# raider99k/UNINA-YOLO-DLA

Measured on NVIDIA B200. Metric: images/sec @640x640 (forward + DFL decode + NMS), higher is better.
Workload: dtype bf16

## Files before the change

unina-yolo-dla_b200/csrc/api.cu:

```cuda
#include <cstdarg>
#include <cstdlib>
#include <memory>
#include <mutex>
#include <set>
#include <utility>

#include "camera.cuh"
#include "common.cuh"

namespace uyd {

static thread_local char g_err[512] = "";

void set_error(const char *fmt, ...) {
  va_list ap;
  va_start(ap, fmt);
  vsnprintf(g_err, sizeof(g_err), fmt, ap);
  va_end(ap);
}

int smem_optin_impl(const void *kernel, int bytes) {
  static std::mutex mu;
  static std::set<std::pair<const void *, int>> done;
  int dev = 0;
// ... 47 lines not shown

struct ClsArgs {
  const __nv_bfloat16 *in;
  float *out;
  const __nv_bfloat16 *wdw;
  const uint32_t *wfrag;
  const float *bias;
  int n, h, w, in_pitch, out_pitch, nc, tiles_x, tiles_y;
};
bool cls_branch_supported(int cin, int mid, int nc, int h, int w, int in_pitch, int in_coff, int out_pitch, int out_coff);
void cls_branch_pack(int cin, int nc, const float *const w[5], const float *const b[5], std::vector<__nv_bfloat16> &wdw,
                     std::vector<uint32_t> &frags, std::vector<float> &bias);
int cls_branch_launch(int cin, const ClsArgs &a, cudaStream_t s);

struct ChainConv;
ChainConv *chain_new();
void chain_delete(ChainConv *);
bool chain_supported(int cin, int n1, int n2, int in_pitch, int in_coff);
size_t chain_w1_bytes(int cin, int n1, bool depthwise);
size_t chain_w2_bytes(int n1, int n2);
void chain_pack_w1(int cin, int n1, bool depthwise, const float *w, void *dst_host);
void chain_pack_w2(int n1, int n2, const float *w, void *dst_host);
int chain_prepare(ChainConv *cc, int cin, int n1, int n2, void *in_base, int in_pitch, int h, int w, int max_batch,
                  void *w1_dev, void *w2_dev, const float *bias1, const float *bias2, int relu2, int final_kind, int nc,
                  const float *w3_dev, const float *bias3_dev, void *out_base, int out_pitch, int out_f32, int a_total,
                  int a_off, int y_ch0, int no, float stride_px, int dw1);
int chain_launch(const ChainConv *cc, int nb, float *y, int sm_count, cudaStream_t s);

struct StemArgs {
  const void *in;
  __nv_bfloat16 *out;
  const uint32_t *wfrag;
  const float *bias;
  int n, ih, iw, oh, ow, out_pitch, u8, pw;
  CamFrames f;
};
bool stem_fused_supported(int c0, int c1, int ih, int iw, int out_pitch, int out_coff);
void stem_fused_pack(const float *w0, const float *b0, const float *w1, const float *b1, const float *w2, const float *b2,
                     std::vector<uint32_t> &frags, std::vector<float> &bias);
int stem_fused_launch(const StemArgs &a, cudaStream_t s);

// ... 21 lines not shown
  std::vector<float> b_host;
  void *w_dev = nullptr;
  float *b_dev = nullptr;
  TcConv *tc = nullptr;
  std::vector<float> m_host;
  float *m_dev = nullptr;
  float out_scale = 0.f;
  int out_kind = 0;
  std::vector<unsigned char> w2_host;
  void *w2_dev = nullptr;
  int nc = 0;
  uyd_chain chain{};
  ChainConv *cc = nullptr;
  std::vector<float> b2_host, w3_host, b3_host;
  float *b2_dev = nullptr, *w3_dev = nullptr, *b3_dev = nullptr;
  bool quant = false;
  int buf = -1, coff = 0, c = 0, out_buf = -1, out_coff = 0;
};

struct uyd_plan {
  uyd_ctx *ctx = nullptr;
  int max_batch = 0;
  bool finalized = false;
  std::vector<Buffer> bufs;
  std::vector<Op> ops;
  std::vector<int> heads, head_strides;
  int reg_max = 16, nc = 0;
  float dfl_amax = 0.f;
  int in_c = 0, in_h = 0, in_w = 0;
  size_t bytes = 0;
// ... 50 lines not shown
}

extern "C" int uyd_plan_destroy(uyd_plan *plan) {
  if (!plan) return UYD_OK;
  uyd::DeviceGuard guard(plan->ctx->device);
  for (Op &o : plan->ops) {
    if (o.w_dev) cudaFree(o.w_dev);
    if (o.b_dev) cudaFree(o.b_dev);
    if (o.m_dev) cudaFree(o.m_dev);
    if (o.w2_dev) cudaFree(o.w2_dev);
    if (o.tc) tc_delete(o.tc);
    if (o.cc) chain_delete(o.cc);
    if (o.b2_dev) cudaFree(o.b2_dev);
    if (o.w3_dev) cudaFree(o.w3_dev);
    if (o.b3_dev) cudaFree(o.b3_dev);
  }
  if (plan->arena) cudaFree(plan->arena);
  for (cudaEvent_t e : plan->timed_ev) cudaEventDestroy(e);
  delete plan;
  return UYD_OK;
}

extern "C" int uyd_plan_add_buffer(uyd_plan *plan, int h, int w, int c, int dtype, int *id) {
  UYD_REQUIRE(plan && id && h > 0 && w > 0 && c > 0, UYD_E_ARG, "uyd_plan_add_buffer: bad arguments");
  UYD_REQUIRE(!plan->finalized, UYD_E_STATE, "plan already finalized");
  UYD_REQUIRE(dtype == UYD_BF16 || dtype == UYD_F32 || dtype == UYD_S8, UYD_E_ARG, "unknown dtype %d", dtype);
  Buffer b;
  b.h = h; b.w = w; b.c = c; b.dtype = dtype;
  plan->bufs.push_back(b);
  *id = (int)plan->bufs.size() - 1;
// ... 372 lines not shown
    UYD_REQUIRE(b.dtype == UYD_F32 && b.c == 4 * reg_max + nc, UYD_E_ARG, "head buffer %d must be fp32 with %d channels", i,
                4 * reg_max + nc);
  }
  plan->heads.assign(head_bufs, head_bufs + nl);
  plan->head_strides.assign(strides, strides + nl);
  plan->reg_max = reg_max;
  plan->nc = nc;
  return UYD_OK;
}

static void *slice_ptr(const uyd_plan *p, int buf, int coff) {
  const Buffer &b = p->bufs[buf];
  return (char *)b.ptr + (size_t)coff * b.elem_bytes();
}

extern "C" int uyd_plan_finalize(uyd_plan *plan) {
  UYD_REQUIRE(plan && !plan->finalized, UYD_E_STATE, "plan missing or already finalized");
  UYD_REQUIRE(!plan->arena, UYD_E_STATE, "uyd_plan_finalize failed before on this plan: destroy it (uyd_plan_destroy frees the partial allocations)");
  uyd::DeviceGuard guard(plan->ctx->device);
  UYD_CUDA(guard.err);
  size_t total = 0;
  std::vector<size_t> offs;
  for (Buffer &b : plan->bufs) {
    offs.push_back(total);
    total += (b.bytes_per_image() * plan->max_batch + 1023) & ~(size_t)1023;
  }
  UYD_CUDA(cudaMalloc(&plan->arena, total ? total : 1024));
  UYD_CUDA(cudaMemset(plan->arena, 0, total ? total : 1024));
  for (size_t i = 0; i < plan->bufs.size(); ++i) plan->bufs[i].ptr = (char *)plan->arena + offs[i];
  plan->bytes = total;
  const int halo_fallback = env_int("UYD_TC_NO_HALO", 0);
  const int bo_mode = env_int("UYD_TC_BASE_OFFSET", 0);
  const int stages = env_int("UYD_TC_STAGES", 0);
  const int halo_pitch = env_int("UYD_TC_HALO_PITCH", 10);
  for (Op &o : plan->ops) {
    if (o.kind != OP_CONV && o.kind != OP_CONV_S8 && o.kind != OP_C3K && o.kind != OP_CLS && o.kind != OP_CHAIN && o.kind != OP_STEM2) continue;
    UYD_CUDA(cudaMalloc(&o.w_dev, o.w_host.size()));
    UYD_CUDA(cudaMemcpy(o.w_dev, o.w_host.data(), o.w_host.size(), cudaMemcpyHostToDevice));
    UYD_CUDA(cudaMalloc((void **)&o.b_dev, o.b_host.size() * 4));
    UYD_CUDA(cudaMemcpy(o.b_dev, o.b_host.data(), o.b_host.size() * 4, cudaMemcpyHostToDevice));
    plan->bytes += o.w_host.size() + o.b_host.size() * 4;
    o.w_host.clear();
    o.w_host.shrink_to_fit();
    if (o.kind == OP_CLS) {
      UYD_CUDA(cudaMalloc(&o.w2_dev, o.w2_host.size()));
      UYD_CUDA(cudaMemcpy(o.w2_dev, o.w2_host.data(), o.w2_host.size(), cudaMemcpyHostToDevice));
      continue;
    }
    if (o.kind == OP_CHAIN) {
      const uyd_chain &d = o.chain;
      UYD_CUDA(cudaMalloc(&o.w2_dev, o.w2_host.size()));
      UYD_CUDA(cudaMemcpy(o.w2_dev, o.w2_host.data(), o.w2_host.size(), cudaMemcpyHostToDevice));
      UYD_CUDA(cudaMalloc((void **)&o.b2_dev, o.b2_host.size() * 4));
      UYD_CUDA(cudaMemcpy(o.b2_dev, o.b2_host.data(), o.b2_host.size() * 4, cudaMemcpyHostToDevice));
      if (!o.w3_host.empty()) {
        UYD_CUDA(cudaMalloc((void **)&o.w3_dev, o.w3_host.size() * 4));
        UYD_CUDA(cudaMemcpy(o.w3_dev, o.w3_host.data(), o.w3_host.size() * 4, cudaMemcpyHostToDevice));
        UYD_CUDA(cudaMalloc((void **)&o.b3_dev, o.b3_host.size() * 4));
        UYD_CUDA(cudaMemcpy(o.b3_dev, o.b3_host.data(), o.b3_host.size() * 4, cudaMemcpyHostToDevice));
      }
      const Buffer &ib = plan->bufs[d.in_buf];
      void *out = nullptr;
      int out_pitch = 0, out_f32 = 0;
      if (d.out_buf >= 0) {
        out = slice_ptr(plan, d.out_buf, d.out_coff);
        out_pitch = plan->bufs[d.out_buf].c;
        out_f32 = plan->bufs[d.out_buf].dtype == UYD_F32;
      }
      o.cc = chain_new();
      int e = chain_prepare(o.cc, d.cin, d.n1, d.n2, slice_ptr(plan, d.in_buf, d.in_coff), ib.c, ib.h, ib.w, plan->max_batch, o.w_dev,
                            o.w2_dev, o.b_dev, o.b2_dev, d.relu2, d.final_kind, d.nc, o.w3_dev, o.b3_dev, out, out_pitch, out_f32,
                            d.a_total, d.a_off, d.y_ch0, d.no, d.stride_px, d.dw1);
      if (e) return e;
      continue;
    }
    if (o.kind == OP_C3K || o.kind == OP_STEM2) continue;
    if (o.kind == OP_CONV_S8) {
      UYD_CUDA(cudaMalloc((void **)&o.m_dev, o.m_host.size() * 4));
      UYD_CUDA(cudaMemcpy(o.m_dev, o.m_host.data(), o.m_host.size() * 4, cudaMemcpyHostToDevice));
      if (o.use_tc) {
        const uyd_conv &d = o.conv;
        const Buffer &ib = plan->bufs[d.in_buf], &ob = plan->bufs[d.out_buf];
        o.tc = tc_new();
        const void *res = d.res_buf >= 0 ? slice_ptr(plan, d.res_buf, d.res_coff) : nullptr;
        int e = tc_prepare(o.tc, d, slice_ptr(plan, d.in_buf, d.in_coff), ib.c, ib.h, ib.w, plan->max_batch,
                           slice_ptr(plan, d.out_buf, d.out_coff), ob.c, 0, res, d.res_buf >= 0 ? plan->bufs[d.res_buf].c : 0, o.w_dev,
                           o.b_dev, halo_fallback ? 2 : -1, bo_mode, stages, 1, o.m_dev, o.out_scale, o.out_kind, halo_pitch);
// ... 269 lines not shown
    by = (double)b.h * b.w * o.c * 3;
    snprintf(text, text_len, "quantize c%d %dx%d bf16->s8", o.c, b.h, b.w);
  } else if (o.kind == OP_STEM2) {
    const Buffer &b = plan->bufs[o.out_buf];
    fl = 2.0 * (4.0 * b.h * b.w * 16 * 27 + (double)b.h * b.w * 32 * 144 + (o.c ? (double)b.h * b.w * 16 * 32 : 0.0));
    by = 16.0 * b.h * b.w * 3 * 4 + (double)b.h * b.w * (o.c ? 16 : 32) * 2;
    snprintf(text, text_len, "stem2 3->16 k3 s2 + 16->32 k3 s2%s fused -> %dx%d", o.c ? " + 32->16 k1" : "", b.h, b.w);
  } else if (o.kind == OP_CHAIN) {
    const uyd_chain &d = o.chain;
    const Buffer &b = plan->bufs[d.in_buf];
    const double px = (double)b.h * b.w;
    fl = 2.0 * px * ((d.dw1 ? 9.0 * d.cin : 9.0 * d.cin * d.n1) + (double)d.n1 * d.n2 + (d.final_kind == UYD_CHAIN_PW3 ? (double)d.n2 * d.nc : 0.0));
    const double dec = d.final_kind == UYD_CHAIN_DFL ? 16 : (d.final_kind == UYD_CHAIN_PW3 ? 4.0 * d.nc : 0);
    const double rawb = d.out_buf >= 0 ? (d.final_kind == UYD_CHAIN_PW3 ? 4.0 * d.nc : d.n2 * (double)plan->bufs[d.out_buf].elem_bytes()) : 0;
    by = px * (d.cin * 2.0 + rawb + (d.out_buf >= 0 && d.final_kind != UYD_CHAIN_STORE ? 0 : dec));
    snprintf(text, text_len, "chain %s%d->%d k3 + %d->%d k1 + %s %dx%d tc", d.dw1 ? "dw" : "", d.cin, d.n1, d.n1, d.n2,
             d.final_kind == UYD_CHAIN_DFL ? "dfl" : (d.final_kind == UYD_CHAIN_PW3 ? "pw3" : "store"), b.h, b.w);
  } else if (o.kind == OP_CLS) {
    const Buffer &b = plan->bufs[o.buf];
    const double c = o.c;
    fl = 2.0 * b.h * b.w * (9 * c + c * 32 + 9 * 32 + 32 * 32 + 32 * o.nc);
    by = (double)b.h * b.w * (c * 2 + o.nc * 4);
    snprintf(text, text_len, "cls_branch_fused c%d %dx%d (5 convs)", o.c, b.h, b.w);
  } else if (o.kind == OP_C3K) {
    const Buffer &b = plan->bufs[o.buf];
    const double c = o.c, h = c / 2;
    fl = 2.0 * b.h * b.w * (2 * c * h + 4 * 9 * h * h + c * c);
    by = (double)b.h * b.w * c * 2 * 2;
    snprintf(text, text_len, "%s c%d %dx%d (7 convs)", o.quant ? "c3k_fused_s8" : "c3k_fused", o.c, b.h, b.w);
  } else if (o.kind == OP_SPPF) {
    const Buffer &b = plan->bufs[o.buf];
    by = (double)b.h * b.w * o.c * 2 * 4;
// ... 52 lines not shown
```

unina-yolo-dla_b200/csrc/conv_chain.cu:

```cuda
#include <cstdlib>

#include "common.cuh"
#include "tc_ptx.cuh"

namespace uyd {

enum { CH_STORE = 0, CH_PW3 = 2, CH_DFL = 3 };

struct ChainParams {
  int H, W, n0, nb;
  int tiles_x, tiles_y;
  long long total_tiles;
  int ncb, cb_bytes;
  int N1, N2;
  int c2;
  int stages;
  uint32_t blk_bytes, tx_bytes, w1_bytes, w2_bytes, a2_bytes;
  uint32_t idesc1, idesc2, layout1, layout2;
  int relu2, final_kind, nc;
  const float *bias1, *bias2, *bias3, *w3;
  const float *dw_w;
  void *out;
  int out_pitch, out_f32;
  float *y;
  int a_total, a_off, y_ch0, no;
  float stride_px;
  unsigned tpi, m_tpi, m_tx;
  long long *dbg;
};

namespace {

constexpr int kNG = 3;
constexpr int kChainThreads = 128 + 128 * kNG;
constexpr int kHaloRows = 18, kTileH = 16, kTileW = 8, kHaloPitch = kTileW + 2;

__device__ __forceinline__ float sigmoidf_(float x) { return __fdividef(1.0f, 1.0f + __expf(-x)); }

__device__ __forceinline__ float2 ffma2(float2 a, float2 b, float2 c) {
  float2 d;
  asm("{\n\t.reg .b64 ra, rb, rc, rd;\n\tmov.b64 ra, {%2, %3};\n\tmov.b64 rb, {%4, %5};\n\tmov.b64 rc, {%6, %7};\n\t"
      "fma.rn.f32x2 rd, ra, rb, rc;\n\tmov.b64 {%0, %1}, rd;\n\t}"
      : "=f"(d.x), "=f"(d.y)
      : "f"(a.x), "f"(a.y), "f"(b.x), "f"(b.y), "f"(c.x), "f"(c.y));
  return d;
}

__device__ __forceinline__ void load_bias16(const float *s, float (&v)[16]) {
#pragma unroll
  for (int i = 0; i < 4; ++i) {
    const float4 q = reinterpret_cast<const float4 *>(s)[i];
    v[4 * i] = q.x; v[4 * i + 1] = q.y; v[4 * i + 2] = q.z; v[4 * i + 3] = q.w;
  }
}

__device__ __forceinline__ void stamp(const ChainParams &p, int it, int slot, int lane) {
  if (p.dbg && blockIdx.x == 0 && lane == 0 && it < 64) p.dbg[(slot >> 3) * 512 + it * 8 + (slot & 7)] = clock64();
}

template <int KS1, int KS2, bool DW>
__global__ void __launch_bounds__(kChainThreads, 1) conv_chain_kernel(const __grid_constant__ CUtensorMap tm_in,
                                                                      const __grid_constant__ CUtensorMap tm_w1,
                                                                      const __grid_constant__ CUtensorMap tm_w2,
                                                                      const ChainParams p) {
  extern __shared__ unsigned char smem_dyn[];
  const uint32_t raw = smem_u32(smem_dyn);
  const uint32_t base = (raw + 1023u) & ~1023u;
  const uint32_t w1_s = base;
  const uint32_t w2_s = w1_s + ((p.w1_bytes + 1023u) & ~1023u);
  const uint32_t a2_s = w2_s + ((p.w2_bytes + 1023u) & ~1023u);
  const uint32_t a_s = a2_s + (uint32_t)kNG * p.a2_bytes;
  const uint32_t bar0 = a_s + (uint32_t)p.stages * p.blk_bytes;
  const uint32_t full0 = bar0, empty0 = bar0 + 64, wfull = bar0 + 128;
  const uint32_t tfull1 = bar0 + 136, tempty1 = bar0 + 168, a2full = bar0 + 200, tfull2 = bar0 + 232, tempty2 = bar0 + 264;
  const uint32_t slot = bar0 + 296;
  uint32_t *slot_ptr = reinterpret_cast<uint32_t *>(smem_dyn + (slot - raw));
  float *fs = reinterpret_cast<float *>(smem_dyn + (bar0 + 320u - raw));
  float *bias1_s = fs, *bias2_s = fs + 128, *bias3_s = fs + 256, *w3_s = fs + 264;

  const int warp = threadIdx.x >> 5, lane = threadIdx.x & 31;
  uint32_t tmem_cols = 32;
  while (tmem_cols < (uint32_t)kNG * (uint32_t)(p.N1 + p.N2)) tmem_cols <<= 1;

  if (threadIdx.x == 0) {
    for (int s = 0; s < p.stages; ++s) {
      mbar_init(full0 + 8u * s, 1);
      mbar_init(empty0 + 8u * s, DW ? 128 : 1);
    }
    mbar_init(wfull, 1);
    for (int g = 0; g < kNG; ++g) {
      mbar_init(tfull1 + 8u * g, 1);
      mbar_init(tempty1 + 8u * g, 128);
      mbar_init(a2full + 8u * g, 128);
      mbar_init(tfull2 + 8u * g, 1);
      mbar_init(tempty2 + 8u * g, 128);
    }
    fence_barrier_init();
    mbar_expect_tx(wfull, p.w1_bytes + p.w2_bytes);
    const int nblk = DW ? 0 : p.ncb * 9;
    for (int i = 0; i < nblk; ++i) tma_load_2d(w1_s + (uint32_t)i * p.N1 * p.cb_bytes, &tm_w1, wfull, 0, i * p.N1);
    tma_load_2d(w2_s, &tm_w2, wfull, 0, 0);
  }
  griddep_trigger();
  for (int i = threadIdx.x; i < 128; i += kChainThreads) {
    bias1_s[i] = i < p.N1 ? p.bias1[i] : 0.f;
    bias2_s[i] = i < p.N2 ? p.bias2[i] : 0.f;
  }
  if (p.final_kind == CH_PW3) {
    for (int i = threadIdx.x; i < 8 * 64; i += kChainThreads) {
      const int k = i >> 3, c = i & 7;
      w3_s[((k >> 1) * 8 + c) * 2 + (k & 1)] = (c < p.nc && k < p.N2) ? p.w3[c * p.N2 + k] : 0.f;
    }
    if (threadIdx.x < 8) bias3_s[threadIdx.x] = threadIdx.x < p.nc ? p.bias3[threadIdx.x] : 0.f;
  }
  if (warp == 1) tmem_alloc(slot, tmem_cols);
  tc_fence_before();
  __syncthreads();
  tc_fence_after();
  const uint32_t tmem_base = *slot_ptr;
  griddep_wait();

  const int stages = p.stages;
  const uint32_t blk_bytes = p.blk_bytes, cb_bytes = p.cb_bytes;
  const uint32_t cb2_bytes = (uint32_t)p.N1 * 2u;

  if (warp == 0) {
    int stage = 0;
    uint32_t phase = 0;
// ... 3 lines not shown
      const unsigned ty = fastdiv(t, (unsigned)p.tiles_x, p.m_tx);
      const int n = p.n0 + (int)img;
      const int y0 = (int)ty * kTileH, x0 = (int)(t - ty * (unsigned)p.tiles_x) * kTileW;
      for (int j = 0; j < p.ncb; ++j) {
        mbar_wait(empty0 + 8u * stage, phase ^ 1u);
        if (lane == 0) {
          const uint32_t fb = full0 + 8u * stage;
          mbar_expect_tx(fb, p.tx_bytes);
          tma_load_4d(a_s + (uint32_t)stage * blk_bytes, &tm_in, fb, j * cb_elems, x0 - 1, y0 - 1, n);
          if (p.dbg && blockIdx.x == 0) { const int itp = (int)((tile - blockIdx.x) / gridDim.x); if (itp < 64) p.dbg[itp * 8 + 0] = clock64(); }
        }
        __syncwarp();
        if (++stage == stages) { stage = 0; phase ^= 1u; }
      }
    }
  } else if (warp == 1 && !DW) {
    mbar_wait(wfull, 0);
    int stage = 0;
    uint32_t phase = 0;
    const uint64_t adesc0 = make_desc_base((uint32_t)kHaloPitch * cb_bytes, p.layout1);
    const uint64_t bdesc0 = make_desc_base(8u * cb_bytes, p.layout1);
    const uint32_t wblk_units = ((uint32_t)p.N1 * cb_bytes) >> 4;
    const uint32_t px_units = cb_bytes >> 4, row_units = (uint32_t)kHaloPitch * px_units;
    int it = 0, g = 0;
    uint32_t gph = 0;
    for (long long tile = blockIdx.x; tile < p.total_tiles; tile += gridDim.x, ++it) {
      mbar_wait(tempty1 + 8u * g, gph ^ 1u);
      const uint32_t d1 = tmem_base + (uint32_t)g * p.N1;
      for (int j = 0; j < p.ncb; ++j) {
        mbar_wait(full0 + 8u * stage, phase);
        tc_fence_after();
        stamp(p, it, 1, lane);
        const uint64_t ablk_d = adesc0 + (uint64_t)(((a_s + (uint32_t)stage * blk_bytes) & 0x3FFFFu) >> 4);
        const uint64_t wd0 = bdesc0 + (uint64_t)(((w1_s + (uint32_t)(j * 9) * p.N1 * cb_bytes) & 0x3FFFFu) >> 4);
        if (elect_one()) {
#pragma unroll
          for (int t = 0; t < 9; ++t) {
            const uint64_t ad = ablk_d + (uint64_t)((t / 3) * row_units + (t % 3) * px_units);
            const uint64_t wd = wd0 + (uint64_t)t * wblk_units;
#pragma unroll
            for (int k = 0; k < KS1; ++k) umma_bf16(d1, ad + 2 * k, wd + 2 * k, p.idesc1, (j != 0 || t != 0 || k != 0) ? 1u : 0u);
          }
          umma_commit(empty0 + 8u * stage);
          if (j == p.ncb - 1) umma_commit(tfull1 + 8u * g);
        }
        __syncwarp();
        if (++stage == stages) { stage = 0; phase ^= 1u; }
      }
      if (++g == kNG) { g = 0; gph ^= 1u; }
// ... 132 lines not shown
              w1[i] = relu_pack_bf16x2(__uint_as_float(cur[8 + 2 * i]) + bv[8 + 2 * i], __uint_as_float(cur[8 + 2 * i + 1]) + bv[8 + 2 * i + 1]);
            }
            *reinterpret_cast<uint4 *>(a2_row + (((uint32_t)(2 * c) ^ swz) << 4)) = o0;
            *reinterpret_cast<uint4 *>(a2_row + (((uint32_t)(2 * c + 1) ^ swz) << 4)) = o1;
            if (more) {
              tmem_ld_wait();
#pragma unroll
              for (int i = 0; i < 16; ++i) cur[i] = nxt[i];
            }
          }
        }
      }
      fence_proxy_async_smem();
      mbar_arrive(a2full + 8u * g);
      if (q == 0) stamp(p, it, 4, lane);
      mbar_wait(tfull2 + 8u * g, ph);
      tc_fence_after();
      if (q == 0) stamp(p, it, 5, lane);
      const uint32_t t2 = lane_base + (uint32_t)kNG * (uint32_t)p.N1 + (uint32_t)g * p.N2;
      const long long pix = ((long long)n * p.H + oy) * p.W + ox;
      const int nch2 = p.N2 >> 4;
      if (p.final_kind == CH_DFL) {
        float d[4];
        uint32_t cur[16], nxt[16];
        tmem_ld16_issue(t2, cur);
        tmem_ld_wait();
#pragma unroll
        for (int side = 0; side < 4; ++side) {
          if (side < 3) {
            tmem_ld16_issue(t2 + 16u * (side + 1), nxt);
          } else {
            tc_fence_before();
            mbar_arrive(tempty2 + 8u * g);
          }
          float v[16];
          load_bias16(bias2_s + side * 16, v);
#pragma unroll
// ... 17 lines not shown
          if (side < 3) {
            tmem_ld_wait();
#pragma unroll
            for (int i = 0; i < 16; ++i) cur[i] = nxt[i];
          }
        }
        if (p.y && inside) {
          const float ax = (float)ox + 0.5f, ay = (float)oy + 0.5f;
          const float x1 = ax - d[0], y1 = ay - d[1], x2 = ax + d[2], y2 = ay + d[3];
          float *yo = p.y + ((long long)n * p.no + p.y_ch0) * p.a_total + p.a_off + oy * p.W + ox;
          yo[0] = (x1 + x2) * 0.5f * p.stride_px;
          yo[(long long)p.a_total] = (y1 + y2) * 0.5f * p.stride_px;
          yo[2ll * p.a_total] = (x2 - x1) * p.stride_px;
          yo[3ll * p.a_total] = (y2 - y1) * p.stride_px;
        }
      } else if (p.final_kind == CH_PW3) {
        float2 acc[8];
#pragma unroll
        for (int c = 0; c < 8; ++c) acc[c] = make_float2(bias3_s[c], 0.f);
        uint32_t cur[16], nxt[16];
        tmem_ld16_issue(t2, cur);
        tmem_ld_wait();
        for (int ch = 0; ch < nch2; ++ch) {
          const bool more = ch + 1 < nch2;
          if (more) {
            tmem_ld16_issue(t2 + 16u * (ch + 1), nxt);
          } else {
            tc_fence_before();
            mbar_arrive(tempty2 + 8u * g);
          }
          float bv[16];
// ... 105 lines not shown
  EncodeTiledFn fn = chain_encode_fn();
  UYD_REQUIRE(fn, UYD_E_NOGPU, "cuTensorMapEncodeTiled is not available (no CUDA driver)");
  const cuuint32_t one4[4] = {1, 1, 1, 1};
  const CUtensorMapSwizzle sw = row_bytes == 128 ? CU_TENSOR_MAP_SWIZZLE_128B
                                                 : (row_bytes == 64 ? CU_TENSOR_MAP_SWIZZLE_64B : CU_TENSOR_MAP_SWIZZLE_32B);
  CUresult r = fn(tm, CU_TENSOR_MAP_DATA_TYPE_BFLOAT16, (cuuint32_t)rank, base, dims, strides_bytes, box, one4,
                  CU_TENSOR_MAP_INTERLEAVE_NONE, sw, CU_TENSOR_MAP_L2_PROMOTION_L2_128B, CU_TENSOR_MAP_FLOAT_OOB_FILL_NONE);
  UYD_REQUIRE(r == CUDA_SUCCESS, UYD_E_ARG, "conv_chain: cuTensorMapEncodeTiled failed with CUresult %d (rank %d)", (int)r, rank);
  return UYD_OK;
}

uint32_t layout_code(int row_bytes) { return row_bytes == 128 ? 2u : (row_bytes == 64 ? 4u : 6u); }

}

struct ChainConv {
  CUtensorMap tm_in, tm_w1, tm_w2;
  ChainParams p;
  size_t smem;
  bool dw = false;
};

ChainConv *chain_new() { return new ChainConv(); }
void chain_delete(ChainConv *c) { delete c; }

bool chain_supported(int cin, int n1, int n2, int in_pitch, int in_coff) {
  if (!(cin == 32 || cin == 64) || !(n1 == 32 || n1 == 64) || n2 < 1 || n2 > 64) return false;
  return in_pitch % 8 == 0 && in_coff % 8 == 0;
}

size_t chain_w1_bytes(int cin, int n1, bool depthwise) { return depthwise ? (size_t)9 * cin * 4 : (size_t)9 * cin * n1 * 2; }
size_t chain_w2_bytes(int n1, int n2) { return (size_t)n1 * ((n2 + 15) / 16 * 16) * 2; }

void chain_pack_w1(int cin, int n1, bool depthwise, const float *w, void *dst_host) {
  if (depthwise) {
// ... 8 lines not shown
      for (int c = 0; c < cin; ++c) {
        o[((size_t)t * n1 + n) * cin + c] = __float2bfloat16_rn(w[((size_t)n * cin + c) * 9 + t]);
      }
}

void chain_pack_w2(int n1, int n2, const float *w, void *dst_host) {
  __nv_bfloat16 *o = reinterpret_cast<__nv_bfloat16 *>(dst_host);
  const int N2 = (n2 + 15) / 16 * 16;
  for (int n = 0; n < N2; ++n)
    for (int k = 0; k < n1; ++k) o[(size_t)n * n1 + k] = __float2bfloat16_rn(n < n2 ? w[(size_t)n * n1 + k] : 0.f);
}

int chain_prepare(ChainConv *cc, int cin, int n1, int n2, void *in_base, int in_pitch, int h, int w, int max_batch,
                  void *w1_dev, void *w2_dev, const float *bias1, const float *bias2, int relu2, int final_kind, int nc,
                  const float *w3_dev, const float *bias3_dev, void *out_base, int out_pitch, int out_f32, int a_total,
                  int a_off, int y_ch0, int no, float stride_px, int dw1) {
  ChainParams &p = cc->p;
  memset(&p, 0, sizeof(p));
  cc->dw = dw1 != 0;
  p.dw_w = dw1 ? reinterpret_cast<const float *>(w1_dev) : nullptr;
  p.H = h; p.W = w;
  p.ncb = 1;
  p.cb_bytes = cin * 2;
  p.N1 = n1;
  p.N2 = (n2 + 15) / 16 * 16;
  p.c2 = n2;
  UYD_REQUIRE(final_kind != CH_DFL || p.N2 == 64, UYD_E_UNSUPPORTED, "conv_chain: the DFL final needs 4 x 16 logits");
  UYD_REQUIRE(final_kind != CH_PW3 || (nc >= 1 && nc <= 8 && w3_dev && bias3_dev), UYD_E_UNSUPPORTED, "conv_chain: PW3 needs nc <= 8");
  p.tiles_x = ceil_div(w, kTileW);
  p.tiles_y = ceil_div(h, kTileH);
  p.tpi = (unsigned)(p.tiles_x * p.tiles_y);
  p.m_tpi = fastdiv_magic(p.tpi);
  p.m_tx = fastdiv_magic((unsigned)p.tiles_x);
  p.blk_bytes = ((uint32_t)kHaloRows * kHaloPitch * p.cb_bytes + 1023u) & ~1023u;
  p.tx_bytes = (uint32_t)kHaloRows * kHaloPitch * p.cb_bytes;
  p.w1_bytes = dw1 ? 0u : (uint32_t)chain_w1_bytes(cin, n1, false);
  p.w2_bytes = (uint32_t)chain_w2_bytes(n1, n2);
  p.a2_bytes = 128u * (uint32_t)n1 * 2u;
  p.layout1 = layout_code(p.cb_bytes);
  p.layout2 = layout_code(n1 * 2);
  p.idesc1 = (1u << 4) | (1u << 7) | (1u << 10) | ((uint32_t)(p.N1 >> 3) << 17) | ((uint32_t)(128 >> 4) << 24);
  p.idesc2 = (1u << 4) | (1u << 7) | (1u << 10) | ((uint32_t)(p.N2 >> 3) << 17) | ((uint32_t)(128 >> 4) << 24);
  p.relu2 = relu2;
  p.final_kind = final_kind;
  p.nc = nc;
  p.bias1 = bias1; p.bias2 = bias2; p.bias3 = bias3_dev; p.w3 = w3_dev;
  p.out = out_base; p.out_pitch = out_pitch; p.out_f32 = out_f32;
  p.a_total = a_total; p.a_off = a_off; p.y_ch0 = y_ch0; p.no = no; p.stride_px = stride_px;
  const size_t fixed = 1024 + ((p.w1_bytes + 1023u) & ~1023u) + ((p.w2_bytes + 1023u) & ~1023u) + (size_t)kNG * p.a2_bytes + 320 + 4096;
  int stages = (int)((227 * 1024 - fixed) / p.blk_bytes);
  UYD_REQUIRE(stages >= 2, UYD_E_UNSUPPORTED, "conv_chain: %d -> %d -> %d leaves no room for two halo stages", cin, n1, n2);
  if (stages > 6) stages = 6;
  p.stages = stages;
  cc->smem = fixed + (size_t)stages * p.blk_bytes;
  if (!dw1) {
    const cuuint64_t dims[2] = {(cuuint64_t)cin, (cuuint64_t)9 * n1};
    const cuuint64_t str[1] = {(cuuint64_t)p.cb_bytes};
    const cuuint32_t box[2] = {(cuuint32_t)cin, (cuuint32_t)n1};
    int e = chain_encode(&cc->tm_w1, w1_dev, 2, dims, str, box, p.cb_bytes);
    if (e) return e;
  } else {
    cc->tm_w1 = cc->tm_w2;
  }
  {
    const cuuint64_t dims[2] = {(cuuint64_t)n1, (cuuint64_t)p.N2};
    const cuuint64_t str[1] = {(cuuint64_t)n1 * 2};
    const cuuint32_t box[2] = {(cuuint32_t)n1, (cuuint32_t)p.N2};
    int e = chain_encode(&cc->tm_w2, w2_dev, 2, dims, str, box, n1 * 2);
    if (e) return e;
  }
  {
    const cuuint64_t dims[4] = {(cuuint64_t)cin, (cuuint64_t)w, (cuuint64_t)h, (cuuint64_t)max_batch};
    const cuuint64_t str[3] = {(cuuint64_t)in_pitch * 2, (cuuint64_t)w * in_pitch * 2, (cuuint64_t)h * w * in_pitch * 2};
    const cuuint32_t box[4] = {(cuuint32_t)cin, (cuuint32_t)kHaloPitch, (cuuint32_t)kHaloRows, 1};
    int e = chain_encode(&cc->tm_in, in_base, 4, dims, str, box, p.cb_bytes);
    if (e) return e;
  }
  if (int e = smem_optin(conv_chain_kernel<2, 2, false>, 227 * 1024)) return e;
  if (int e = smem_optin(conv_chain_kernel<2, 4, false>, 227 * 1024)) return e;
  if (int e = smem_optin(conv_chain_kernel<4, 2, false>, 227 * 1024)) return e;
  if (int e = smem_optin(conv_chain_kernel<4, 4, false>, 227 * 1024)) return e;
  if (int e = smem_optin(conv_chain_kernel<2, 2, true>, 227 * 1024)) return e;
  if (int e = smem_optin(conv_chain_kernel<4, 4, true>, 227 * 1024)) return e;
  return UYD_OK;
}

int chain_launch(const ChainConv *cc, int nb, float *y, int sm_count, cudaStream_t s) {
  ChainParams p = cc->p;
  p.n0 = 0;
  p.nb = nb;
  p.y = y;
  p.total_tiles = (long long)nb * p.tiles_x * p.tiles_y;
  if (p.total_tiles == 0) return UYD_OK;
  UYD_REQUIRE(p.total_tiles < (1ll << 31), UYD_E_UNSUPPORTED, "conv_chain: %lld tiles exceed the kernel's 32-bit tile index", p.total_tiles);
  const unsigned grid = (unsigned)(p.total_tiles < sm_count ? p.total_tiles : sm_count);
  const int ks1 = p.cb_bytes / 32, ks2 = p.N1 * 2 / 32;
#ifdef UYD_CHAIN_TIMELINE_BUILD
  static long long *dbg_dev = nullptr;
  const bool timeline = getenv("UYD_CHAIN_TIMELINE") && p.total_tiles >= 64ll * grid;
  if (timeline) {
    if (!dbg_dev) cudaMalloc(&dbg_dev, 2 * 64 * 8 * sizeof(long long));
    cudaMemsetAsync(dbg_dev, 0, 2 * 64 * 8 * sizeof(long long), s);
    p.dbg = dbg_dev;
  }
#endif
#define UYD_CHAIN_LAUNCH(A, B, D) UYD_CUDA(launch_pdl(conv_chain_kernel<A, B, D>, dim3(grid), dim3(kChainThreads), cc->smem, s, cc->tm_in, cc->tm_w1, cc->tm_w2, p))
  if (cc->dw) {
    if (ks1 == 2) UYD_CHAIN_LAUNCH(2, 2, true);
    else UYD_CHAIN_LAUNCH(4, 4, true);
  } else if (ks1 == 2 && ks2 == 2) UYD_CHAIN_LAUNCH(2, 2, false);
  else if (ks1 == 2 && ks2 == 4) UYD_CHAIN_LAUNCH(2, 4, false);
  else if (ks1 == 4 && ks2 == 2) UYD_CHAIN_LAUNCH(4, 2, false);
  else UYD_CHAIN_LAUNCH(4, 4, false);
#undef UYD_CHAIN_LAUNCH
#ifdef UYD_CHAIN_TIMELINE_BUILD
  if (timeline) {
    long long h[2 * 64 * 8];
    cudaStreamSynchronize(s);
    cudaMemcpy(h, dbg_dev, sizeof(h), cudaMemcpyDeviceToHost);
    fprintf(stderr, "chain timeline cin=%d N1=%d N2=%d final=%d (tma g1issue g2issue acc1 a2 acc2 done)\n", p.cb_bytes / 2, p.N1, p.N2, p.final_kind);
    for (int t = 0; t < 40; ++t) {
      fprintf(stderr, "  tile %2d:", t);
// ... 12 lines not shown
```

Measured before the change: 32880.

## Pair head box 3x3 conv with depthwise class chain sharing the input halo

Adds a plan pass that merges a standalone 3x3 64-output box-branch conv with a later depthwise STORE chain that reads the same input slice. The merged chain kernel runs the dense conv's 9-tap GEMM on the otherwise idle MMA warp, using the same TMA halo stages. Extra TMEM columns hold its accumulator, and the epilogue warps apply bias and ReLU and write bf16 output. This removes one kernel launch and a second read of the head input, at the cost of more TMEM and shared memory per CTA and a longer epilogue in the chain kernel.

Result: faster. 33440 (median of 6 runs) (+1.7%).

```diff
diff --git a/unina-yolo-dla_b200/csrc/api.cu b/unina-yolo-dla_b200/csrc/api.cu
--- a/unina-yolo-dla_b200/csrc/api.cu
+++ b/unina-yolo-dla_b200/csrc/api.cu
@@ -1,4 +1,5 @@
 #include <cstdarg>
+#include <algorithm>
 #include <cstdlib>
 #include <memory>
 #include <mutex>
@@ -85,6 +86,12 @@
 int cls_branch_launch(int cin, const ClsArgs &a, cudaStream_t s);
 
 struct ChainConv;
+struct ChainBox {
+  void *w_dev;
+  const float *bias;
+  void *out;
+  int out_pitch;
+};
 ChainConv *chain_new();
 void chain_delete(ChainConv *);
 bool chain_supported(int cin, int n1, int n2, int in_pitch, int in_coff);
@@ -95,7 +102,7 @@
 int chain_prepare(ChainConv *cc, int cin, int n1, int n2, void *in_base, int in_pitch, int h, int w, int max_batch,
                   void *w1_dev, void *w2_dev, const float *bias1, const float *bias2, int relu2, int final_kind, int nc,
                   const float *w3_dev, const float *bias3_dev, void *out_base, int out_pitch, int out_f32, int a_total,
-                  int a_off, int y_ch0, int no, float stride_px, int dw1);
+                  int a_off, int y_ch0, int no, float stride_px, int dw1, const ChainBox *box);
 int chain_launch(const ChainConv *cc, int nb, float *y, int sm_count, cudaStream_t s);
 
 struct StemArgs {
@@ -147,6 +154,11 @@
   ChainConv *cc = nullptr;
   std::vector<float> b2_host, w3_host, b3_host;
   float *b2_dev = nullptr, *w3_dev = nullptr, *b3_dev = nullptr;
+  bool paired = false;
+  std::vector<unsigned char> wc_host;
+  std::vector<float> bc_host;
+  void *wc_dev = nullptr;
+  float *bc_dev = nullptr;
   bool quant = false;
   int buf = -1, coff = 0, c = 0, out_buf = -1, out_coff = 0;
 };
@@ -227,6 +239,8 @@
     if (o.b2_dev) cudaFree(o.b2_dev);
     if (o.w3_dev) cudaFree(o.w3_dev);
     if (o.b3_dev) cudaFree(o.b3_dev);
+    if (o.wc_dev) cudaFree(o.wc_dev);
+    if (o.bc_dev) cudaFree(o.bc_dev);
   }
   if (plan->arena) cudaFree(plan->arena);
   for (cudaEvent_t e : plan->timed_ev) cudaEventDestroy(e);
@@ -629,6 +643,74 @@
   return (char *)b.ptr + (size_t)coff * b.elem_bytes();
 }
 
+static void op_buffers(const Op &o, std::vector<int> &rd, std::vector<int> &wr) {
+  rd.clear();
+  wr.clear();
+  switch (o.kind) {
+    case OP_CONV:
+    case OP_CONV_S8:
+      rd = {o.conv.in_buf, o.conv.res_buf, o.conv.pre_buf_p1 - 1};
+      wr = {o.conv.out_buf};
+      break;
+    case OP_CHAIN:
+      rd = {o.chain.in_buf};
+      wr = {o.chain.out_buf};
+      if (o.paired) wr.push_back(o.conv.out_buf);
+      break;
+    case OP_STEM2:
+      wr = {o.out_buf};
+      break;
+    case OP_SPPF:
+      rd = {o.buf};
+      wr = {o.buf};
+      break;
+    default:
+      rd = {o.buf};
+      wr = {o.out_buf};
+      break;
+  }
+}
+
+static void pair_head_convs(uyd_plan *plan, bool halo_off) {
+  if (env_int("UYD_NO_HEAD_PAIR", 0) || halo_off) return;
+  std::vector<Op> &ops = plan->ops;
+  std::vector<int> rd, wr;
+  auto has = [](const std::vector<int> &v, int b) { return b >= 0 && std::find(v.begin(), v.end(), b) != v.end(); };
+  for (size_t i = 0; i < ops.size(); ++i) {
+    const Op &c = ops[i];
+    const uyd_conv &d = c.conv;
+    if (c.kind != OP_CONV || !c.use_tc || d.k != 3 || d.stride != 1 || d.depthwise || !d.relu || d.res_buf >= 0 || d.pre_buf_p1 ||
+        d.in_buf < 0 || d.cout != 64 || !(d.cin == 32 || d.cin == 64) || plan->bufs[d.out_buf].dtype != UYD_BF16 ||
+        d.out_buf == d.in_buf)
+      continue;
+    for (size_t j = i + 1; j < ops.size(); ++j) {
+      const Op &h = ops[j];
+      const uyd_chain &ch = h.chain;
+      if (h.kind == OP_CHAIN && !h.paired && ch.dw1 && ch.final_kind == UYD_CHAIN_STORE && ch.in_buf == d.in_buf &&
+          ch.in_coff == d.in_coff && ch.cin == d.cin && 3 * (ch.n1 + (ch.n2 + 15) / 16 * 16 + 64) <= 512 &&
+          ch.out_buf != d.in_buf && ch.out_buf != d.out_buf) {
+        bool ok = true;
+        for (size_t k = i + 1; k < j && ok; ++k) {
+          op_buffers(ops[k], rd, wr);
+          ok = !has(wr, d.in_buf) && !has(wr, ch.out_buf) && !has(rd, ch.out_buf);
+        }
+        if (ok) {
+          Op m = std::move(ops[j]);
+          m.paired = true;
+          m.conv = d;
+          m.wc_host = std::move(ops[i].w_host);
+          m.bc_host = std::move(ops[i].b_host);
+          ops.erase(ops.begin() + j);
+          ops[i] = std::move(m);
+        }
+        break;
+      }
+      op_buffers(h, rd, wr);
+      if (has(wr, d.in_buf)) break;
+    }
+  }
+}
+
 extern "C" int uyd_plan_finalize(uyd_plan *plan) {
   UYD_REQUIRE(plan && !plan->finalized, UYD_E_STATE, "plan missing or already finalized");
   UYD_REQUIRE(!plan->arena, UYD_E_STATE, "uyd_plan_finalize failed before on this plan: destroy it (uyd_plan_destroy frees the partial allocations)");
@@ -648,6 +730,7 @@
   const int bo_mode = env_int("UYD_TC_BASE_OFFSET", 0);
   const int stages = env_int("UYD_TC_STAGES", 0);
   const int halo_pitch = env_int("UYD_TC_HALO_PITCH", 10);
+  pair_head_convs(plan, halo_fallback != 0);
   for (Op &o : plan->ops) {
     if (o.kind != OP_CONV && o.kind != OP_CONV_S8 && o.kind != OP_C3K && o.kind != OP_CLS && o.kind != OP_CHAIN && o.kind != OP_STEM2) continue;
     UYD_CUDA(cudaMalloc(&o.w_dev, o.w_host.size()));
@@ -674,6 +757,20 @@
         UYD_CUDA(cudaMalloc((void **)&o.b3_dev, o.b3_host.size() * 4));
         UYD_CUDA(cudaMemcpy(o.b3_dev, o.b3_host.data(), o.b3_host.size() * 4, cudaMemcpyHostToDevice));
       }
+      ChainBox box{};
+      if (o.paired) {
+        UYD_CUDA(cudaMalloc(&o.wc_dev, o.wc_host.size()));
+        UYD_CUDA(cudaMemcpy(o.wc_dev, o.wc_host.data(), o.wc_host.size(), cudaMemcpyHostToDevice));
+        UYD_CUDA(cudaMalloc((void **)&o.bc_dev, o.bc_host.size() * 4));
+        UYD_CUDA(cudaMemcpy(o.bc_dev, o.bc_host.data(), o.bc_host.size() * 4, cudaMemcpyHostToDevice));
+        plan->bytes += o.wc_host.size() + o.bc_host.size() * 4;
+        o.wc_host.clear();
+        o.wc_host.shrink_to_fit();
+        box.w_dev = o.wc_dev;
+        box.bias = o.bc_dev;
+        box.out = slice_ptr(plan, o.conv.out_buf, o.conv.out_coff);
+        box.out_pitch = plan->bufs[o.conv.out_buf].c;
+      }
       const Buffer &ib = plan->bufs[d.in_buf];
       void *out = nullptr;
       int out_pitch = 0, out_f32 = 0;
@@ -685,7 +782,7 @@
       o.cc = chain_new();
       int e = chain_prepare(o.cc, d.cin, d.n1, d.n2, slice_ptr(plan, d.in_buf, d.in_coff), ib.c, ib.h, ib.w, plan->max_batch, o.w_dev,
                             o.w2_dev, o.b_dev, o.b2_dev, d.relu2, d.final_kind, d.nc, o.w3_dev, o.b3_dev, out, out_pitch, out_f32,
-                            d.a_total, d.a_off, d.y_ch0, d.no, d.stride_px, d.dw1);
+                            d.a_total, d.a_off, d.y_ch0, d.no, d.stride_px, d.dw1, o.paired ? &box : nullptr);
       if (e) return e;
       continue;
     }
@@ -985,8 +1082,15 @@
     const double dec = d.final_kind == UYD_CHAIN_DFL ? 16 : (d.final_kind == UYD_CHAIN_PW3 ? 4.0 * d.nc : 0);
     const double rawb = d.out_buf >= 0 ? (d.final_kind == UYD_CHAIN_PW3 ? 4.0 * d.nc : d.n2 * (double)plan->bufs[d.out_buf].elem_bytes()) : 0;
     by = px * (d.cin * 2.0 + rawb + (d.out_buf >= 0 && d.final_kind != UYD_CHAIN_STORE ? 0 : dec));
-    snprintf(text, text_len, "chain %s%d->%d k3 + %d->%d k1 + %s %dx%d tc", d.dw1 ? "dw" : "", d.cin, d.n1, d.n1, d.n2,
-             d.final_kind == UYD_CHAIN_DFL ? "dfl" : (d.final_kind == UYD_CHAIN_PW3 ? "pw3" : "store"), b.h, b.w);
+    const char *fin = d.final_kind == UYD_CHAIN_DFL ? "dfl" : (d.final_kind == UYD_CHAIN_PW3 ? "pw3" : "store");
+    if (o.paired) {
+      fl += 2.0 * px * 9.0 * o.conv.cin * o.conv.cout;
+      by += px * o.conv.cout * 2.0;
+      snprintf(text, text_len, "chain %s%d->%d k3 + %d->%d k1 + %s | conv %d->%d k3 %dx%d tc", d.dw1 ? "dw" : "", d.cin, d.n1, d.n1, d.n2,
+               fin, o.conv.cin, o.conv.cout, b.h, b.w);
+    } else {
+      snprintf(text, text_len, "chain %s%d->%d k3 + %d->%d k1 + %s %dx%d tc", d.dw1 ? "dw" : "", d.cin, d.n1, d.n1, d.n2, fin, b.h, b.w);
+    }
   } else if (o.kind == OP_CLS) {
     const Buffer &b = plan->bufs[o.buf];
     const double c = o.c;
diff --git a/unina-yolo-dla_b200/csrc/conv_chain.cu b/unina-yolo-dla_b200/csrc/conv_chain.cu
--- a/unina-yolo-dla_b200/csrc/conv_chain.cu
+++ b/unina-yolo-dla_b200/csrc/conv_chain.cu
@@ -27,6 +27,9 @@
   float stride_px;
   unsigned tpi, m_tpi, m_tx;
   long long *dbg;
+  const float *box_bias;
+  __nv_bfloat16 *box_out;
+  int box_pitch;
 };
 
 namespace {
@@ -34,6 +37,7 @@
 constexpr int kNG = 3;
 constexpr int kChainThreads = 128 + 128 * kNG;
 constexpr int kHaloRows = 18, kTileH = 16, kTileW = 8, kHaloPitch = kTileW + 2;
+constexpr int kBoxN = 64;
 
 __device__ __forceinline__ float sigmoidf_(float x) { return __fdividef(1.0f, 1.0f + __expf(-x)); }
 
@@ -58,11 +62,12 @@
   if (p.dbg && blockIdx.x == 0 && lane == 0 && it < 64) p.dbg[(slot >> 3) * 512 + it * 8 + (slot & 7)] = clock64();
 }
 
-template <int KS1, int KS2, bool DW>
+template <int KS1, int KS2, bool DW, bool PAIR = false>
 __global__ void __launch_bounds__(kChainThreads, 1) conv_chain_kernel(const __grid_constant__ CUtensorMap tm_in,
                                                                       const __grid_constant__ CUtensorMap tm_w1,
                                                                       const __grid_constant__ CUtensorMap tm_w2,
                                                                       const ChainParams p) {
+  static_assert(DW || !PAIR, "PAIR runs the box conv next to the depth-wise stage");
   extern __shared__ unsigned char smem_dyn[];
   const uint32_t raw = smem_u32(smem_dyn);
   const uint32_t base = (raw + 1023u) & ~1023u;
@@ -77,15 +82,16 @@
   uint32_t *slot_ptr = reinterpret_cast<uint32_t *>(smem_dyn + (slot - raw));
   float *fs = reinterpret_cast<float *>(smem_dyn + (bar0 + 320u - raw));
   float *bias1_s = fs, *bias2_s = fs + 128, *bias3_s = fs + 256, *w3_s = fs + 264;
+  float *boxb_s = fs + 776;
 
   const int warp = threadIdx.x >> 5, lane = threadIdx.x & 31;
   uint32_t tmem_cols = 32;
-  while (tmem_cols < (uint32_t)kNG * (uint32_t)(p.N1 + p.N2)) tmem_cols <<= 1;
+  while (tmem_cols < (uint32_t)kNG * (uint32_t)(p.N1 + p.N2 + (PAIR ? kBoxN : 0))) tmem_cols <<= 1;
 
   if (threadIdx.x == 0) {
     for (int s = 0; s < p.stages; ++s) {
       mbar_init(full0 + 8u * s, 1);
-      mbar_init(empty0 + 8u * s, DW ? 128 : 1);
+      mbar_init(empty0 + 8u * s, DW ? (PAIR ? 129 : 128) : 1);
     }
     mbar_init(wfull, 1);
     for (int g = 0; g < kNG; ++g) {
@@ -97,8 +103,12 @@
     }
     fence_barrier_init();
     mbar_expect_tx(wfull, p.w1_bytes + p.w2_bytes);
-    const int nblk = DW ? 0 : p.ncb * 9;
-    for (int i = 0; i < nblk; ++i) tma_load_2d(w1_s + (uint32_t)i * p.N1 * p.cb_bytes, &tm_w1, wfull, 0, i * p.N1);
+    if constexpr (PAIR) {
+      for (int i = 0; i < 9; ++i) tma_load_2d(w1_s + (uint32_t)i * kBoxN * p.cb_bytes, &tm_w1, wfull, 0, i * kBoxN);
+    } else {
+      const int nblk = DW ? 0 : p.ncb * 9;
+      for (int i = 0; i < nblk; ++i) tma_load_2d(w1_s + (uint32_t)i * p.N1 * p.cb_bytes, &tm_w1, wfull, 0, i * p.N1);
+    }
     tma_load_2d(w2_s, &tm_w2, wfull, 0, 0);
   }
   griddep_trigger();
@@ -112,6 +122,9 @@
       w3_s[((k >> 1) * 8 + c) * 2 + (k & 1)] = (c < p.nc && k < p.N2) ? p.w3[c * p.N2 + k] : 0.f;
     }
     if (threadIdx.x < 8) bias3_s[threadIdx.x] = threadIdx.x < p.nc ? p.bias3[threadIdx.x] : 0.f;
+  }
+  if constexpr (PAIR) {
+    if (threadIdx.x < kBoxN) boxb_s[threadIdx.x] = p.box_bias[threadIdx.x];
   }
   if (warp == 1) tmem_alloc(slot, tmem_cols);
   tc_fence_before();
@@ -145,25 +158,27 @@
         if (++stage == stages) { stage = 0; phase ^= 1u; }
       }
     }
-  } else if (warp == 1 && !DW) {
+  } else if (warp == 1 && (!DW || PAIR)) {
+    const uint32_t n1 = PAIR ? (uint32_t)kBoxN : (uint32_t)p.N1;
+    const uint32_t d1_0 = tmem_base + (PAIR ? (uint32_t)kNG * (uint32_t)(p.N1 + p.N2) : 0u);
     mbar_wait(wfull, 0);
     int stage = 0;
     uint32_t phase = 0;
     const uint64_t adesc0 = make_desc_base((uint32_t)kHaloPitch * cb_bytes, p.layout1);
     const uint64_t bdesc0 = make_desc_base(8u * cb_bytes, p.layout1);
-    const uint32_t wblk_units = ((uint32_t)p.N1 * cb_bytes) >> 4;
+    const uint32_t wblk_units = (n1 * cb_bytes) >> 4;
     const uint32_t px_units = cb_bytes >> 4, row_units = (uint32_t)kHaloPitch * px_units;
     int it = 0, g = 0;
     uint32_t gph = 0;
     for (long long tile = blockIdx.x; tile < p.total_tiles; tile += gridDim.x, ++it) {
       mbar_wait(tempty1 + 8u * g, gph ^ 1u);
-      const uint32_t d1 = tmem_base + (uint32_t)g * p.N1;
+      const uint32_t d1 = d1_0 + (uint32_t)g * n1;
       for (int j = 0; j < p.ncb; ++j) {
         mbar_wait(full0 + 8u * stage, phase);
         tc_fence_after();
         stamp(p, it, 1, lane);
         const uint64_t ablk_d = adesc0 + (uint64_t)(((a_s + (uint32_t)stage * blk_bytes) & 0x3FFFFu) >> 4);
-        const uint64_t wd0 = bdesc0 + (uint64_t)(((w1_s + (uint32_t)(j * 9) * p.N1 * cb_bytes) & 0x3FFFFu) >> 4);
+        const uint64_t wd0 = bdesc0 + (uint64_t)(((w1_s + (uint32_t)(j * 9) * n1 * cb_bytes) & 0x3FFFFu) >> 4);
         if (elect_one()) {
 #pragma unroll
           for (int t = 0; t < 9; ++t) {
@@ -326,13 +341,49 @@
       fence_proxy_async_smem();
       mbar_arrive(a2full + 8u * g);
       if (q == 0) stamp(p, it, 4, lane);
+      if constexpr (PAIR) {
+        mbar_wait(tfull1 + 8u * g, ph);
+        tc_fence_after();
+        const uint32_t tb = lane_base + (uint32_t)kNG * (uint32_t)(p.N1 + p.N2) + (uint32_t)g * kBoxN;
+        uint4 *bo = reinterpret_cast<uint4 *>(p.box_out + (((long long)n * p.H + oy) * p.W + ox) * p.box_pitch);
+        uint32_t cur[16], nxt[16];
+        tmem_ld16_issue(tb, cur);
+        tmem_ld_wait();
+#pragma unroll
+        for (int c = 0; c < kBoxN / 16; ++c) {
+          if (c + 1 < kBoxN / 16) {
+            tmem_ld16_issue(tb + 16u * (c + 1), nxt);
+          } else {
+            tc_fence_before();
+            mbar_arrive(tempty1 + 8u * g);
+          }
+          if (inside) {
+            float bv[16];
+            load_bias16(boxb_s + c * 16, bv);
+            uint4 o0, o1;
+            uint32_t *w0 = reinterpret_cast<uint32_t *>(&o0), *w1 = reinterpret_cast<uint32_t *>(&o1);
+#pragma unroll
+            for (int i = 0; i < 4; ++i) {
+              w0[i] = relu_pack_bf16x2(__uint_as_float(cur[2 * i]) + bv[2 * i], __uint_as_float(cur[2 * i + 1]) + bv[2 * i + 1]);
+              w1[i] = relu_pack_bf16x2(__uint_as_float(cur[8 + 2 * i]) + bv[8 + 2 * i], __uint_as_float(cur[8 + 2 * i + 1]) + bv[8 + 2 * i + 1]);
+            }
+            bo[2 * c] = o0;
+            bo[2 * c + 1] = o1;
+          }
+          if (c + 1 < kBoxN / 16) {
+            tmem_ld_wait();
+#pragma unroll
+            for (int i = 0; i < 16; ++i) cur[i] = nxt[i];
+          }
+        }
+      }
       mbar_wait(tfull2 + 8u * g, ph);
       tc_fence_after();
       if (q == 0) stamp(p, it, 5, lane);
       const uint32_t t2 = lane_base + (uint32_t)kNG * (uint32_t)p.N1 + (uint32_t)g * p.N2;
       const long long pix = ((long long)n * p.H + oy) * p.W + ox;
       const int nch2 = p.N2 >> 4;
-      if (p.final_kind == CH_DFL) {
+      if (!PAIR && p.final_kind == CH_DFL) {
         float d[4];
         uint32_t cur[16], nxt[16];
         tmem_ld16_issue(t2, cur);
@@ -380,7 +431,7 @@
           yo[2ll * p.a_total] = (x2 - x1) * p.stride_px;
           yo[3ll * p.a_total] = (y2 - y1) * p.stride_px;
         }
-      } else if (p.final_kind == CH_PW3) {
+      } else if (!PAIR && p.final_kind == CH_PW3) {
         float2 acc[8];
 #pragma unroll
         for (int c = 0; c < 8; ++c) acc[c] = make_float2(bias3_s[c], 0.f);
@@ -516,11 +567,19 @@
 
 }
 
+struct ChainBox {
+  void *w_dev;
+  const float *bias;
+  void *out;
+  int out_pitch;
+};
+
 struct ChainConv {
   CUtensorMap tm_in, tm_w1, tm_w2;
   ChainParams p;
   size_t smem;
   bool dw = false;
+  bool pair = false;
 };
 
 ChainConv *chain_new() { return new ChainConv(); }
@@ -559,10 +618,11 @@
 int chain_prepare(ChainConv *cc, int cin, int n1, int n2, void *in_base, int in_pitch, int h, int w, int max_batch,
                   void *w1_dev, void *w2_dev, const float *bias1, const float *bias2, int relu2, int final_kind, int nc,
                   const float *w3_dev, const float *bias3_dev, void *out_base, int out_pitch, int out_f32, int a_total,
-                  int a_off, int y_ch0, int no, float stride_px, int dw1) {
+                  int a_off, int y_ch0, int no, float stride_px, int dw1, const ChainBox *box) {
   ChainParams &p = cc->p;
   memset(&p, 0, sizeof(p));
   cc->dw = dw1 != 0;
+  cc->pair = box != nullptr;
   p.dw_w = dw1 ? reinterpret_cast<const float *>(w1_dev) : nullptr;
   p.H = h; p.W = w;
   p.ncb = 1;
@@ -572,6 +632,8 @@
   p.c2 = n2;
   UYD_REQUIRE(final_kind != CH_DFL || p.N2 == 64, UYD_E_UNSUPPORTED, "conv_chain: the DFL final needs 4 x 16 logits");
   UYD_REQUIRE(final_kind != CH_PW3 || (nc >= 1 && nc <= 8 && w3_dev && bias3_dev), UYD_E_UNSUPPORTED, "conv_chain: PW3 needs nc <= 8");
+  UYD_REQUIRE(!box || (dw1 && final_kind == CH_STORE && kNG * (n1 + p.N2 + kBoxN) <= 512), UYD_E_UNSUPPORTED,
+              "conv_chain: a box conv pairs with a depth-wise STORE chain whose accumulators fit 512 TMEM columns");
   p.tiles_x = ceil_div(w, kTileW);
   p.tiles_y = ceil_div(h, kTileH);
   p.tpi = (unsigned)(p.tiles_x * p.tiles_y);
@@ -579,12 +641,13 @@
   p.m_tx = fastdiv_magic((unsigned)p.tiles_x);
   p.blk_bytes = ((uint32_t)kHaloRows * kHaloPitch * p.cb_bytes + 1023u) & ~1023u;
   p.tx_bytes = (uint32_t)kHaloRows * kHaloPitch * p.cb_bytes;
-  p.w1_bytes = dw1 ? 0u : (uint32_t)chain_w1_bytes(cin, n1, false);
+  p.w1_bytes = box ? (uint32_t)chain_w1_bytes(cin, kBoxN, false) : (dw1 ? 0u : (uint32_t)chain_w1_bytes(cin, n1, false));
   p.w2_bytes = (uint32_t)chain_w2_bytes(n1, n2);
   p.a2_bytes = 128u * (uint32_t)n1 * 2u;
   p.layout1 = layout_code(p.cb_bytes);
   p.layout2 = layout_code(n1 * 2);
-  p.idesc1 = (1u << 4) | (1u << 7) | (1u << 10) | ((uint32_t)(p.N1 >> 3) << 17) | ((uint32_t)(128 >> 4) << 24);
+  const int gemm1_n = box ? kBoxN : p.N1;
+  p.idesc1 = (1u << 4) | (1u << 7) | (1u << 10) | ((uint32_t)(gemm1_n >> 3) << 17) | ((uint32_t)(128 >> 4) << 24);
   p.idesc2 = (1u << 4) | (1u << 7) | (1u << 10) | ((uint32_t)(p.N2 >> 3) << 17) | ((uint32_t)(128 >> 4) << 24);
   p.relu2 = relu2;
   p.final_kind = final_kind;
@@ -592,17 +655,24 @@
   p.bias1 = bias1; p.bias2 = bias2; p.bias3 = bias3_dev; p.w3 = w3_dev;
   p.out = out_base; p.out_pitch = out_pitch; p.out_f32 = out_f32;
   p.a_total = a_total; p.a_off = a_off; p.y_ch0 = y_ch0; p.no = no; p.stride_px = stride_px;
+  if (box) {
+    UYD_REQUIRE(box->out_pitch % 8 == 0 && (reinterpret_cast<uintptr_t>(box->out) & 15) == 0, UYD_E_UNSUPPORTED,
+                "conv_chain: the box conv's output rows must be 16-byte aligned");
+    p.box_bias = box->bias;
+    p.box_out = reinterpret_cast<__nv_bfloat16 *>(box->out);
+    p.box_pitch = box->out_pitch;
+  }
   const size_t fixed = 1024 + ((p.w1_bytes + 1023u) & ~1023u) + ((p.w2_bytes + 1023u) & ~1023u) + (size_t)kNG * p.a2_bytes + 320 + 4096;
   int stages = (int)((227 * 1024 - fixed) / p.blk_bytes);
   UYD_REQUIRE(stages >= 2, UYD_E_UNSUPPORTED, "conv_chain: %d -> %d -> %d leaves no room for two halo stages", cin, n1, n2);
   if (stages > 6) stages = 6;
   p.stages = stages;
   cc->smem = fixed + (size_t)stages * p.blk_bytes;
-  if (!dw1) {
-    const cuuint64_t dims[2] = {(cuuint64_t)cin, (cuuint64_t)9 * n1};
+  if (!dw1 || box) {
+    const cuuint64_t dims[2] = {(cuuint64_t)cin, (cuuint64_t)9 * gemm1_n};
     const cuuint64_t str[1] = {(cuuint64_t)p.cb_bytes};
-    const cuuint32_t box[2] = {(cuuint32_t)cin, (cuuint32_t)n1};
-    int e = chain_encode(&cc->tm_w1, w1_dev, 2, dims, str, box, p.cb_bytes);
+    const cuuint32_t boxdim[2] = {(cuuint32_t)cin, (cuuint32_t)gemm1_n};
+    int e = chain_encode(&cc->tm_w1, box ? box->w_dev : w1_dev, 2, dims, str, boxdim, p.cb_bytes);
     if (e) return e;
   } else {
     cc->tm_w1 = cc->tm_w2;
@@ -627,6 +697,8 @@
   if (int e = smem_optin(conv_chain_kernel<4, 4, false>, 227 * 1024)) return e;
   if (int e = smem_optin(conv_chain_kernel<2, 2, true>, 227 * 1024)) return e;
   if (int e = smem_optin(conv_chain_kernel<4, 4, true>, 227 * 1024)) return e;
+  if (int e = smem_optin(conv_chain_kernel<2, 2, true, true>, 227 * 1024)) return e;
+  if (int e = smem_optin(conv_chain_kernel<4, 4, true, true>, 227 * 1024)) return e;
   return UYD_OK;
 }
 
@@ -649,8 +721,11 @@
     p.dbg = dbg_dev;
   }
 #endif
-#define UYD_CHAIN_LAUNCH(A, B, D) UYD_CUDA(launch_pdl(conv_chain_kernel<A, B, D>, dim3(grid), dim3(kChainThreads), cc->smem, s, cc->tm_in, cc->tm_w1, cc->tm_w2, p))
-  if (cc->dw) {
+#define UYD_CHAIN_LAUNCH(A, B, ...) UYD_CUDA(launch_pdl(conv_chain_kernel<A, B, __VA_ARGS__>, dim3(grid), dim3(kChainThreads), cc->smem, s, cc->tm_in, cc->tm_w1, cc->tm_w2, p))
+  if (cc->pair) {
+    if (ks1 == 2) UYD_CHAIN_LAUNCH(2, 2, true, true);
+    else UYD_CHAIN_LAUNCH(4, 4, true, true);
+  } else if (cc->dw) {
     if (ks1 == 2) UYD_CHAIN_LAUNCH(2, 2, true);
     else UYD_CHAIN_LAUNCH(4, 4, true);
   } else if (ks1 == 2 && ks2 == 2) UYD_CHAIN_LAUNCH(2, 2, false);
```
